# pratyushkumar211/industrial_nnmpc_2021

Hardware: NVIDIA B200
Metric: cdu_closed_loop_sim_steps_per_s (higher is better)
Workload: dtype f64

## Files before the change

industrial_nnmpc_2021_b200/csrc/oz.cu:

```cuda
#include "oz_gemm.cuh"
#include "oz.cuh"
#include "lp.cuh"
#include <cstdlib>
#include <cstring>

namespace nnmpc {

constexpr int OZ_LMAX = 7;
constexpr int OZ_NS = OZ_LMAX + 1;
#ifndef NNMPC_OZ_LMAX_ANCHOR
#define NNMPC_OZ_LMAX_ANCHOR 5
#endif
constexpr int OZ_LMAX_ANCHOR = NNMPC_OZ_LMAX_ANCHOR;

static int oz_variant() {
  static int v = -1;
  if (v < 0) {
    const char* e = getenv("NNMPC_OZ_VARIANT");
    v = e ? atoi(e) : 2;
    if (v < 0 || v > 3) v = 2;
  }
  return v;
}

struct OzEpiStore {
  struct Params {
    double* C;
    long long ldc;
  };
  Params p;
  long long pos;
  __device__ explicit OzEpiStore(const Params& p_) : p(p_), pos(0) {}
  __device__ void begin_row(int pos_, bool) { pos = pos_; }
  __device__ void chunk(int col0, const double (&v)[oz::CH], int N) {
#pragma unroll
    for (int k = 0; k < oz::CH; ++k)
      if (col0 + k < N) p.C[pos * p.ldc + col0 + k] = v[k];
  }
  __device__ void end_row() {}
};

struct OzEpiAnchor {
  struct Params {
    double* X;
    const double* C;
    const int* rows;
    int n;
  };
  Params p;
  long long base;
  __device__ explicit OzEpiAnchor(const Params& p_) : p(p_), base(0) {}
  __device__ void begin_row(int pos, bool ok) { base = ok ? (long long)(p.rows ? p.rows[pos] : pos) * p.n : 0; }
  __device__ void chunk(int col0, const double (&v)[oz::CH], int N) {
    double2 c[oz::CH / 2];
#pragma unroll
    for (int k = 0; k < oz::CH; k += 2) {
      const int col = col0 + k;
      c[k / 2] = make_double2(0.0, 0.0);
      if (col + 1 < N) c[k / 2] = *reinterpret_cast<const double2*>(p.C + base + col);
      else if (col < N) c[k / 2].x = p.C[base + col];
    }
#pragma unroll
    for (int k = 0; k < oz::CH; k += 2) {
      const int col = col0 + k;
      if (col + 1 < N) *reinterpret_cast<double2*>(p.X + base + col) = make_double2(v[k] - c[k / 2].x, v[k + 1] - c[k / 2].y);
      else if (col < N) p.X[base + col] = v[k] - c[k / 2].x;
    }
  }
  __device__ void end_row() {}
};

struct OzEpiVerify {
  struct Params {
    const double* Z;
    const double* Ql;
    const double* lb;
    const double* ub;
    unsigned long long* kres;
    double* G;
    const int* rows;
    int n, nu;
  };
  Params p;
  long long pr;
  bool ok;
  double rmax;
  __device__ explicit OzEpiVerify(const Params& p_) : p(p_), pr(0), ok(false), rmax(0.0) {}
  __device__ void begin_row(int pos, bool ok_) {
    ok = ok_;
    pr = ok ? (long long)(p.rows ? p.rows[pos] : pos) : 0;
    rmax = 0.0;
  }
  __device__ void chunk(int col0, const double (&v)[oz::CH], int N) {
    const long long base = pr * p.n;
    const double* lbr = p.lb + pr * p.nu;
    const double* ubr = p.ub + pr * p.nu;
#pragma unroll
    for (int h = 0; h < oz::CH; h += oz::CH / 2) {
      double z[oz::CH / 2], ql[oz::CH / 2], l[oz::CH / 2], u[oz::CH / 2];
#pragma unroll
      for (int k = 0; k < oz::CH / 2; ++k) {
        const int col = col0 + h + k;
        const bool in = col < N;
        const int s = (in ? col : 0) % p.nu;
        z[k] = in ? p.Z[base + col] : 0.0;
        ql[k] = in ? p.Ql[base + col] : 0.0;
        l[k] = lbr[s];
        u[k] = ubr[s];
      }
#pragma unroll
      for (int k = 0; k < oz::CH / 2; ++k) {
        const int col = col0 + h + k;
        if (col < N) {
          const double g = v[h + k] + ql[k];
          if (p.G) p.G[base + col] = g;
          double r = fabs(z[k] - fmin(fmax(z[k] - g, l[k]), u[k]));
          if (!(r <= 1.7e308)) r = __longlong_as_double(0x7ff0000000000000ll);
          rmax = fmax(rmax, r);
        }
      }
    }
  }
  __device__ void end_row() {
    if (ok) atomicMax(p.kres + pr, (unsigned long long)__double_as_longlong(rmax));
  }
};

int oz_slice_operator(const double* T_dev, int nrows, int ncols, OzOperator* op, cudaStream_t st, long long ld) {
  if (ncols > 32768) return set_error(NNMPC_ERR_BADARG, "oz_slice_operator: contraction length %d above 32768 (int32 accumulators)", ncols);
  op->nrows = nrows; op->ncols = ncols;
  op->ldb = ((long long)ncols + oz::BKB - 1) / oz::BKB * oz::BKB;
  op->rows_pad = ((long long)nrows + 127) / 128 * 128;
  const size_t bytes = (size_t)OZ_NS * op->rows_pad * op->ldb;
  NNMPC_TRY(op->S.ensure(bytes));
  NNMPC_TRY(op->escale.ensure((size_t)op->rows_pad));
  NNMPC_CUDA(cudaMemsetAsync(op->S.p, 0, bytes, st));
  NNMPC_CUDA(cudaMemsetAsync(op->escale.p, 0, (size_t)op->rows_pad * sizeof(double), st));
  oz::k_oz_slice<OZ_NS><<<nrows, 256, 0, st>>>(nullptr, nullptr, T_dev, ld > 0 ? ld : ncols, ncols, op->S.p, op->rows_pad,
                                               op->ldb, op->escale.p, nrows);
  count_launch();
  NNMPC_CUDA(cudaGetLastError());
  if (!oz::make_tmap_u8(&op->tm, op->S.p, OZ_NS * op->rows_pad, op->ldb, op->ldb, oz::BN))
    return set_error(NNMPC_ERR_CUDA, "cuTensorMapEncodeTiled failed for the operator digit planes");
  if (!oz::make_tmap_u8(&op->tm128, op->S.p, OZ_NS * op->rows_pad, op->ldb, op->ldb, 128))
    return set_error(NNMPC_ERR_CUDA, "cuTensorMapEncodeTiled failed for the operator digit planes");
  op->ready = true;
  return 0;
}

int oz_rows_ensure(OzRows* r, long long cap, int ncols, cudaStream_t st, int ns) {
  if (ns <= 0) ns = OZ_NS;
  const long long ldb = ((long long)ncols + oz::BKB - 1) / oz::BKB * oz::BKB;
  const long long cap_pad = (cap + oz::BM - 1) / oz::BM * oz::BM;
  if (cap_pad <= r->cap_pad && ldb == r->ldb && ncols == r->ncols && ns == r->ns) return 0;
  const long long cp = cap_pad > r->cap_pad ? cap_pad : r->cap_pad;
  const size_t bytes = (size_t)ns * cp * ldb;
  NNMPC_TRY(r->S.ensure(bytes));
  NNMPC_TRY(r->fscale.ensure((size_t)cp));
  NNMPC_CUDA(cudaMemsetAsync(r->S.p, 0, bytes, st));
  NNMPC_CUDA(cudaMemsetAsync(r->fscale.p, 0, (size_t)cp * sizeof(double), st));
  if (!oz::make_tmap_u8(&r->tm, r->S.p, ns * cp, ldb, ldb, oz::BM))
    return set_error(NNMPC_ERR_CUDA, "cuTensorMapEncodeTiled failed for the sample digit planes");
  r->cap_pad = cp; r->ldb = ldb; r->ncols = ncols; r->ns = ns;
  return 0;
}

static int oz_slice_rows(OzRows* r, const int* rows, const int* count, int max_rows, const double* src, long long ld_src,
                         cudaStream_t st) {
  if (r->ns == 4 && !rows && !count && r->ncols <= 4096)
    oz::k_oz_slice_warp<4><<<row_grid((max_rows + 7) / 8), 256, 0, st>>>(src, ld_src, r->ncols, r->S.p, r->cap_pad, r->ldb,
                                                                         r->fscale.p, max_rows);
  else if (r->ns == 4)
    oz::k_oz_slice<4><<<row_grid(max_rows), 256, 0, st>>>(rows, count, src, ld_src, r->ncols, r->S.p, r->cap_pad, r->ldb,
                                                          r->fscale.p, max_rows);
  else
    oz::k_oz_slice<OZ_NS><<<row_grid(max_rows), 256, 0, st>>>(rows, count, src, ld_src, r->ncols, r->S.p, r->cap_pad, r->ldb,
                                                              r->fscale.p, max_rows);
  count_launch();
  NNMPC_CUDA(cudaGetLastError());
  return 0;
}

static oz::OzShape oz_shape(const OzOperator* op, const OzRows* r, int max_rows, const int* count) {
  oz::OzShape g{};
  g.M = max_rows; g.N = op->nrows; g.KB = (int)(op->ldb / oz::BKB); g.m_dev = count;
  g.a_rows_pad = r->cap_pad; g.b_rows_pad = op->rows_pad; g.fscale = r->fscale.p; g.escale = op->escale.p;
  g.group_rows = 8;
  return g;
}

template <int LMAX, class Epi>
static int oz_apply(const OzOperator* op, OzRows* r, int max_rows, const int* count, const typename Epi::Params& ep,
                    int device, cudaStream_t st) {
  const int sms = device_sm_count(device);
  const oz::OzShape g = oz_shape(op, r, max_rows, count);
  cudaError_t e;
  const int var = oz_variant();
  if (var == 0) {
    e = oz::launch_oz_gemm<LMAX, Epi>(r->tm, op->tm, g, ep, sms, st);
    count_launch();
  } else if (var == 1) {
    e = oz::launch_oz_gemm2<0, LMAX, 64, Epi>(r->tm, op->tm, oz::OzShape2{g, nullptr, 0, 0}, ep, sms, st);
    count_launch();
  } else {
    NNMPC_TRY(r->partial.ensure((size_t)r->cap_pad * op->nrows));
    e = oz::launch_oz_gemm2<4, LMAX, 128, OzEpiStore>(r->tm, op->tm128, oz::OzShape2{g, nullptr, 0, 1},
                                                      OzEpiStore::Params{r->partial.p, op->nrows}, sms, st);
    if (e == cudaSuccess)
      e = var == 3 ? oz::launch_oz_gemm2<0, 3, 64, Epi>(r->tm, op->tm, oz::OzShape2{g, r->partial.p, op->nrows, 0}, ep, sms, st)
                   : oz::launch_oz_gemm2<0, 3, 128, Epi>(r->tm, op->tm128, oz::OzShape2{g, r->partial.p, op->nrows, 0}, ep, sms, st);
    count_launch(2);
  }
  if (e != cudaSuccess) return set_error(NNMPC_ERR_CUDA, "oz_gemm launch failed: %s", cudaGetErrorString(e));
  return 0;
}

int oz_anchor(const OzOperator* top, OzRows* r, const int* rows, const int* count, int max_rows, const double* W,
              const double* C, double* X, int n, int device, cudaStream_t st) {
  if (max_rows <= 0) return 0;
  if (!top->ready || top->ncols != n || r->ncols != n || max_rows > r->cap_pad)
    return set_error(NNMPC_ERR_BADARG, "oz_anchor: operator / row planes not prepared for n = %d, %d rows", n, max_rows);
  NNMPC_TRY(oz_slice_rows(r, rows, count, max_rows, W, n, st));
  return oz_apply<OZ_LMAX_ANCHOR, OzEpiAnchor>(top, r, max_rows, count, OzEpiAnchor::Params{X, C, rows, n}, device, st);
}

int oz_verify(const OzOperator* P, OzRows* r, const int* rows, const int* count, int max_rows, const double* Z,
              const double* Ql, const double* lb, const double* ub, unsigned long long* kres, double* G, int n, int nu,
              int device, cudaStream_t st) {
  if (max_rows <= 0) return 0;
  if (!P->ready || P->ncols != n || r->ncols != n || max_rows > r->cap_pad)
    return set_error(NNMPC_ERR_BADARG, "oz_verify: operator / row planes not prepared for n = %d, %d rows", n, max_rows);
  NNMPC_TRY(oz_slice_rows(r, rows, count, max_rows, Z, n, st));
  return oz_apply<OZ_LMAX, OzEpiVerify>(P, r, max_rows, count, OzEpiVerify::Params{Z, Ql, lb, ub, kres, G, rows, n, nu},
                                        device, st);
}

struct OzEpiDense {
  struct Params {
    double* out;
    long long ldo;
    const double* bias;
    int relu;
  };
  Params p;
  long long pos;
  __device__ explicit OzEpiDense(const Params& p_) : p(p_), pos(0) {}
  __device__ void begin_row(int pos_, bool) { pos = pos_; }
  __device__ void chunk(int col0, const double (&v)[oz::CH], int N) {
#pragma unroll
    for (int k = 0; k < oz::CH; ++k) {
      const int col = col0 + k;
      if (col < N) {
        double h = v[k] + (p.bias ? __ldg(p.bias + col) : 0.0);
        if (p.relu) h = h > 0.0 ? h : 0.0;
        p.out[pos * p.ldo + col] = h;
      }
    }
  }
  __device__ void end_row() {}
};

int oz_dense_layer(const OzOperator* W, OzRows* r, int M, const double* A, long long lda, const double* bias, int relu,
                   double* out, long long ldo, int device, cudaStream_t st) {
  if (M <= 0) return 0;
  if (!W->ready) return set_error(NNMPC_ERR_BADARG, "oz_dense_layer: weights not sliced");
  NNMPC_TRY(oz_rows_ensure(r, M, W->ncols, st, 4));
  NNMPC_TRY(oz_slice_rows(r, nullptr, nullptr, M, A, lda, st));
  const oz::OzShape g = oz_shape(W, r, M, nullptr);
  cudaError_t e = oz::launch_oz_gemm2<0, 3, 64, OzEpiDense>(r->tm, W->tm, oz::OzShape2{g, nullptr, 0, 0},
                                                            OzEpiDense::Params{out, ldo, bias, relu},
                                                            device_sm_count(device), st);
  count_launch();
  if (e != cudaSuccess) return set_error(NNMPC_ERR_CUDA, "oz_gemm launch failed: %s", cudaGetErrorString(e));
  return 0;
}

struct OzEpiDenseF32 {
  struct Params {
    float* H;
    long long ldh;
    const double* bias;
    float* amax_out;
  };
  Params p;
  long long pos;
  float hmax;
  __device__ explicit OzEpiDenseF32(const Params& p_) : p(p_), pos(0), hmax(0.f) {}
  __device__ void begin_row(int pos_, bool) {
    pos = pos_;
    hmax = 0.f;
  }
  __device__ void chunk(int col0, const double (&v)[oz::CH], int N) {
    __align__(16) float h[oz::CH];
#pragma unroll
    for (int k = 0; k < oz::CH; ++k) {
      double t = 0.0;
      if (col0 + k < N) {
        t = v[k] + __ldg(p.bias + col0 + k);
        t = t > 0.0 ? t : 0.0;
      }
      h[k] = (float)t;
      hmax = fmaxf(hmax, h[k]);
    }
    float4* dst = reinterpret_cast<float4*>(p.H + pos * p.ldh + col0);
#pragma unroll
    for (int q = 0; q < oz::CH / 4; ++q) dst[q] = reinterpret_cast<const float4*>(h)[q];
  }
  __device__ void end_row() {
    atomicMax(reinterpret_cast<unsigned int*>(p.amax_out + pos), __float_as_uint(hmax));
  }
};

__global__ void __launch_bounds__(256)
k_oz_slice_f32(const float* __restrict__ H, long long ldh, int ncols, const float* __restrict__ amax, int8_t* __restrict__ dst,
               long long rows_pad, long long ldb, double* __restrict__ fscale, long long nrows) {
  const int lane = threadIdx.x & 31;
  const long long wpg = (long long)gridDim.x * (blockDim.x >> 5);
  for (long long p = (long long)blockIdx.x * (blockDim.x >> 5) + (threadIdx.x >> 5); p < nrows; p += wpg) {
    const float* a = H + p * ldh;
    const double m = (double)amax[p];
    const bool bad = !(m <= 1.7e308);
    int ex = 0;
    if (!bad && m > 0.0) frexp(m, &ex);
    const double inv = bad ? 0.0 : ldexp(1.0, -(ex + 1));
    for (int k = 4 * lane; k < ncols; k += 128) {
      const float4 f = *reinterpret_cast<const float4*>(a + k);
      double t[4] = {f.x * inv, f.y * inv, f.z * inv, f.w * inv};
#pragma unroll
      for (int s = 0; s < 4; ++s) {
        char4 d;
        int8_t* dd = reinterpret_cast<int8_t*>(&d);
#pragma unroll
        for (int e = 0; e < 4; ++e) {
          t[e] *= 128.0;
          const double r = rint(t[e]);
          t[e] -= r;
          dd[e] = (k + e < ncols) ? (int8_t)(int)r : (int8_t)0;
        }
        *reinterpret_cast<char4*>(dst + ((long long)s * rows_pad + p) * ldb + k) = d;
      }
    }
    if (lane == 0) fscale[p] = bad ? __longlong_as_double(0x7ff8000000000000ll) : ldexp(1.0, ex + 1);
  }
}

int oz_dense_planes(const OzOperator* W, OzRows* rin, int M, const double* bias, OzRows* rout, float* hbuf, long long ldh,
                    float* amax_out, double* out, long long ldo, int device, cudaStream_t st) {
  if (M <= 0) return 0;
  if (!W->ready || rin->ns != 4 || rin->ncols != W->ncols || M > rin->cap_pad)
    return set_error(NNMPC_ERR_BADARG, "oz_dense_planes: operands not prepared");
  const oz::OzShape g = oz_shape(W, rin, M, nullptr);
  cudaError_t e;
  if (out) {
    e = oz::launch_oz_gemm2<0, 3, 64, OzEpiDense>(rin->tm, W->tm, oz::OzShape2{g, nullptr, 0, 0},
                                                  OzEpiDense::Params{out, ldo, bias, 0}, device_sm_count(device), st);
    count_launch();
  } else {
    if (rout->ns != 4 || rout->ncols != W->nrows || M > rout->cap_pad || (ldh & 3) || ldh < ((W->nrows + 63) / 64) * 64)
      return set_error(NNMPC_ERR_BADARG, "oz_dense_planes: output planes / fp32 scratch not prepared");
    e = oz::launch_oz_gemm2<0, 3, 64, OzEpiDenseF32>(rin->tm, W->tm, oz::OzShape2{g, nullptr, 0, 0},
                                                     OzEpiDenseF32::Params{hbuf, ldh, bias, amax_out}, device_sm_count(device), st);
    if (e == cudaSuccess) {
      k_oz_slice_f32<<<row_grid((M + 7) / 8), 256, 0, st>>>(hbuf, ldh, W->nrows, amax_out, rout->S.p, rout->cap_pad, rout->ldb,
                                                            rout->fscale.p, M);
      e = cudaGetLastError();
    }
    count_launch(2);
  }
  if (e != cudaSuccess) return set_error(NNMPC_ERR_CUDA, "oz_gemm launch failed: %s", cudaGetErrorString(e));
  return 0;
}

__global__ void __launch_bounds__(256)
k_oz_pack_network_input(const double* __restrict__ x, const double* __restrict__ uprev, const double* __restrict__ xs,
                        const double* __restrict__ us, const double* __restrict__ xscale, int8_t* __restrict__ dst,
                        long long rows_pad, long long ldb, double* __restrict__ fscale, float* __restrict__ amax, long long B,
                        int nx, int nu, int with_uprev) {
  const int lane = threadIdx.x & 31;
  const long long wpg = (long long)gridDim.x * (blockDim.x >> 5);
  const int o1 = nx, o2 = nx + (with_uprev ? nu : 0), o3 = o2 + nx, o4 = o3 + nu;
  for (long long b = (long long)blockIdx.x * (blockDim.x >> 5) + (threadIdx.x >> 5); b < B; b += wpg) {
    auto value = [&](int c, double& v1, double& v2) {
      if (c < o1) {
        v1 = x[b * nx + c];
        v2 = xs[b * nx + c];
        if (xscale) { v1 /= xscale[c]; v2 /= xscale[c]; }
      } else if (c < o2) {
        v1 = uprev[b * nu + (c - o1)];
        v2 = us[b * nu + (c - o1)];
      } else if (c < o3) {
        v1 = xs[b * nx + (c - o2)];
        if (xscale) v1 /= xscale[c - o2];
        v2 = v1;
      } else {
        v1 = v2 = us[b * nu + (c - o3)];
      }
    };
    double m1 = 0.0, m2 = 0.0;
    for (int c = lane; c < o4; c += 32) {
      double v1, v2;
      value(c, v1, v2);
      const double a1 = fabs(v1), a2 = fabs(v2);
      m1 = (a1 <= m1) ? m1 : a1;
      m2 = (a2 <= m2) ? m2 : a2;
    }
#pragma unroll
    for (int o = 16; o > 0; o >>= 1) {
      const double a1 = __shfl_xor_sync(0xffffffffu, m1, o), a2 = __shfl_xor_sync(0xffffffffu, m2, o);
      m1 = (a1 <= m1) ? m1 : a1;
      m2 = (a2 <= m2) ? m2 : a2;
    }
    double inv[2], fs[2];
    const double mm[2] = {m1, m2};
#pragma unroll
    for (int r = 0; r < 2; ++r) {
      const bool bad = !(mm[r] <= 1.7e308);
      int ex = 0;
      if (!bad && mm[r] > 0.0) frexp(mm[r], &ex);
      inv[r] = bad ? 0.0 : ldexp(1.0, -(ex + 1));
      fs[r] = bad ? __longlong_as_double(0x7ff8000000000000ll) : ldexp(1.0, ex + 1);
    }
    for (int c = lane; c < o4; c += 32) {
      double v1, v2;
      value(c, v1, v2);
      double t1 = v1 * inv[0], t2 = v2 * inv[1];
#pragma unroll
      for (int s = 0; s < 4; ++s) {
        t1 *= 128.0; t2 *= 128.0;
        const double r1 = rint(t1), r2 = rint(t2);
        t1 -= r1; t2 -= r2;
        dst[((long long)s * rows_pad + 2 * b) * ldb + c] = (int8_t)(int)r1;
        dst[((long long)s * rows_pad + 2 * b + 1) * ldb + c] = (int8_t)(int)r2;
      }
    }
    if (lane == 0) {
      fscale[2 * b] = fs[0]; fscale[2 * b + 1] = fs[1];
      amax[2 * b] = (float)m1 * 1.0000002f; amax[2 * b + 1] = (float)m2 * 1.0000002f;
    }
  }
}

int oz_pack_network_input(OzRows* r, long long B, const double* x, const double* uprev, const double* xs, const double* us,
                          const double* xscale, int nx, int nu, int with_uprev, float* amax, cudaStream_t st) {
  if (B <= 0) return 0;
  if (r->ns != 4 || 2 * B > r->cap_pad) return set_error(NNMPC_ERR_BADARG, "oz_pack_network_input: planes not prepared");
  k_oz_pack_network_input<<<row_grid((B + 7) / 8), 256, 0, st>>>(x, uprev, xs, us, xscale, r->S.p, r->cap_pad, r->ldb, r->fscale.p,
                                                                 amax, B, nx, nu, with_uprev);
  count_launch();
  NNMPC_CUDA(cudaGetLastError());
  return 0;
}

}

using namespace nnmpc;

extern "C" {

int nnmpc_oz_gemm_test(int M, int N, int K, const double* A, const double* Bt, double* C, void* stream) {
  if (!A || !Bt || !C || M <= 0 || N <= 0 || K <= 0) return set_error(NNMPC_ERR_BADARG, "nnmpc_oz_gemm_test: bad argument");
  cudaStream_t st = (cudaStream_t)stream;
  int dev = 0;
  NNMPC_CUDA(cudaGetDevice(&dev));
  OzOperator op;
  OzRows rows;
  int rc = oz_slice_operator(Bt, N, K, &op, st);
  if (rc == 0) rc = oz_rows_ensure(&rows, M, K, st);
  if (rc == 0) rc = oz_slice_rows(&rows, nullptr, nullptr, M, A, K, st);
  if (rc == 0) rc = oz_apply<OZ_LMAX, OzEpiStore>(&op, &rows, M, nullptr, OzEpiStore::Params{C, N}, dev, st);
  if (rc == 0 && cudaStreamSynchronize(st) != cudaSuccess)
    rc = set_error(NNMPC_ERR_CUDA, "oz_gemm failed: %s", cudaGetErrorString(cudaGetLastError()));
  cudaStreamSynchronize(st);
  op.release();
  rows.release();
  return rc;
}

int nnmpc_oz_gemm_bench(int M, int N, int K, const double* A, const double* Bt, double* C, int reps, float* ms) {
  if (!A || !Bt || !C || !ms || M <= 0 || N <= 0 || K <= 0 || reps <= 0)
    return set_error(NNMPC_ERR_BADARG, "nnmpc_oz_gemm_bench: bad argument");
  cudaStream_t st = 0;
  int dev = 0;
  NNMPC_CUDA(cudaGetDevice(&dev));
  OzOperator op;
  OzRows rows;
  int rc = oz_slice_operator(Bt, N, K, &op, st);
  if (rc == 0) rc = oz_rows_ensure(&rows, M, K, st);
  cudaEvent_t e0, e1, e2;
  cudaEventCreate(&e0); cudaEventCreate(&e1); cudaEventCreate(&e2);
  for (int w = 0; w < 2 && rc == 0; ++w) {
    rc = oz_slice_rows(&rows, nullptr, nullptr, M, A, K, st);
    if (rc == 0) rc = oz_apply<OZ_LMAX, OzEpiStore>(&op, &rows, M, nullptr, OzEpiStore::Params{C, N}, dev, st);
  }
  if (rc == 0) {
    cudaEventRecord(e0, st);
    for (int i = 0; i < reps && rc == 0; ++i) rc = oz_slice_rows(&rows, nullptr, nullptr, M, A, K, st);
    cudaEventRecord(e1, st);
    for (int i = 0; i < reps && rc == 0; ++i)
      rc = oz_apply<OZ_LMAX, OzEpiStore>(&op, &rows, M, nullptr, OzEpiStore::Params{C, N}, dev, st);
    cudaEventRecord(e2, st);
    if (cudaEventSynchronize(e2) != cudaSuccess) rc = set_error(NNMPC_ERR_CUDA, "oz bench failed: %s", cudaGetErrorString(cudaGetLastError()));
    if (rc == 0) {
      cudaEventElapsedTime(&ms[0], e0, e1);
      cudaEventElapsedTime(&ms[1], e1, e2);
      ms[0] /= reps; ms[1] /= reps;
    }
  }
  cudaEventDestroy(e0); cudaEventDestroy(e1); cudaEventDestroy(e2);
  cudaStreamSynchronize(st);
  op.release();
  rows.release();
  return rc;
}

}
```

industrial_nnmpc_2021_b200/csrc/oz_gemm.cuh:

```cuda
#pragma once
#include "lp_gemm.cuh"

namespace nnmpc {
namespace oz {

constexpr int BM = 128;
constexpr int BN = 64;
constexpr int BKB = 128;
constexpr int UMMA_KB = 32;
constexpr int NS_MAX = 8;
constexpr int A_SLOTS = 4;
constexpr int B_STAGES = 2;
constexpr int A_TILE = BM * BKB;
constexpr int B_TILE = BN * BKB;
constexpr int THREADS = 192;
constexpr int TMEM_COLS = 512;
constexpr int CH = 16;
constexpr int SMEM_BYTES = A_SLOTS * A_TILE + B_STAGES * NS_MAX * B_TILE + 1024 + 256;
static_assert(SMEM_BYTES <= 227 * 1024, "shared memory");

__host__ __device__ constexpr uint32_t make_idesc_i8(int M, int N) {
  return (2u << 4) | (1u << 7) | (1u << 10) | ((uint32_t)(N >> 3) << 17) | ((uint32_t)(M >> 4) << 24);
}
__device__ __forceinline__ void umma_i8(uint32_t tmem_d, uint64_t adesc, uint64_t bdesc, uint32_t idesc, uint32_t accumulate) {
  asm volatile(
      "{\n\t.reg .pred p;\n\t"
      "setp.ne.b32 p, %4, 0;\n\t"
      "tcgen05.mma.cta_group::1.kind::i8 [%0], %1, %2, %3, p;\n\t}"
      ::"r"(tmem_d), "l"(adesc), "l"(bdesc), "r"(idesc), "r"(accumulate)
      : "memory");
}

struct OzShape {
  int M;
  int N;
  int KB;
  const int* m_dev;
  long long a_rows_pad;
  long long b_rows_pad;
  const double* fscale;
  const double* escale;
  int group_rows;
};

__device__ __forceinline__ void oz_tile_coords(int t, int ntm, int ntn, int group_rows, int& bm, int& bn) {
  if (group_rows <= 0 || group_rows >= ntm) {
    bn = t / ntm;
    bm = t - bn * ntm;
    return;
  }
  const int per_group = group_rows * ntn;
  const int gi = t / per_group;
  const int rem = t - gi * per_group;
  const int r0 = gi * group_rows;
  const int gr = (ntm - r0 < group_rows) ? ntm - r0 : group_rows;
  bn = rem / gr;
  bm = r0 + (rem - bn * gr);
}

template <int LMAX, class Epi>
__global__ void __launch_bounds__(THREADS, 1)
oz_gemm_kernel(const __grid_constant__ CUtensorMap tmA, const __grid_constant__ CUtensorMap tmB, OzShape g,
               typename Epi::Params ep) {
  constexpr int NS = LMAX + 1;
  static_assert(NS <= NS_MAX && NS * BN <= TMEM_COLS, "levels");
  extern __shared__ uint8_t smem_raw[];
  uint8_t* base = reinterpret_cast<uint8_t*>((reinterpret_cast<uintptr_t>(smem_raw) + 1023) & ~(uintptr_t)1023);
  uint8_t* a_ring = base;
  uint8_t* b_sets = base + A_SLOTS * A_TILE;
  uint64_t* bars = reinterpret_cast<uint64_t*>(b_sets + B_STAGES * NS_MAX * B_TILE);
  uint64_t* a_full = bars;
  uint64_t* a_empty = a_full + A_SLOTS;
  uint64_t* b_full = a_empty + A_SLOTS;
  uint64_t* b_empty = b_full + B_STAGES;
  uint64_t* acc_full = b_empty + B_STAGES;
  uint64_t* acc_empty = acc_full + 1;
  uint32_t* tmem_slot = reinterpret_cast<uint32_t*>(acc_empty + 1);

  const int warp = threadIdx.x >> 5, lane = threadIdx.x & 31;
  const int M = g.m_dev ? min(*g.m_dev, g.M) : g.M;
  const int ntn = (g.N + BN - 1) / BN;
  const int ntm = (M + BM - 1) / BM;
  const int tiles = ntn * ntm;

  if (warp == 0 && lane == 0) {
    lp::tma_prefetch_desc(&tmA);
    lp::tma_prefetch_desc(&tmB);
    for (int s = 0; s < A_SLOTS; ++s) {
      lp::mbar_init(a_full + s, 1);
      lp::mbar_init(a_empty + s, 1);
    }
    for (int s = 0; s < B_STAGES; ++s) {
      lp::mbar_init(b_full + s, 1);
      lp::mbar_init(b_empty + s, 1);
    }
    lp::mbar_init(acc_full, 1);
    lp::mbar_init(acc_empty, 4);
    lp::fence_barrier_init();
  }
  if (warp == 1) lp::tmem_alloc(tmem_slot, TMEM_COLS);
  lp::tc_fence_before();
  __syncthreads();
  lp::tc_fence_after();
  const uint32_t tmem_base = *tmem_slot;

  if (warp == 0) {
    if (lane == 0) {
      int as = 0, bs = 0;
      uint32_t aph = 0, bph = 0;
      for (int t = blockIdx.x; t < tiles; t += gridDim.x) {
        int bm, bn;
        oz_tile_coords(t, ntm, ntn, g.group_rows, bm, bn);
        for (int kb = 0; kb < g.KB; ++kb) {
          lp::mbar_wait(b_empty + bs, bph ^ 1);
          lp::mbar_expect_tx(b_full + bs, NS * B_TILE);
          for (int j = 0; j < NS; ++j)
            lp::tma_load_2d_hint(b_sets + (bs * NS_MAX + j) * B_TILE, &tmB, b_full + bs, kb * BKB,
                                 (int)(j * g.b_rows_pad) + bn * BN, lp::L2_EVICT_LAST);
          if (++bs == B_STAGES) { bs = 0; bph ^= 1; }
          for (int i = LMAX; i >= 0; --i) {
            lp::mbar_wait(a_empty + as, aph ^ 1);
            lp::mbar_expect_tx(a_full + as, A_TILE);
            lp::tma_load_2d(a_ring + as * A_TILE, &tmA, a_full + as, kb * BKB, (int)(i * g.a_rows_pad) + bm * BM);
            if (++as == A_SLOTS) { as = 0; aph ^= 1; }
          }
        }
      }
    }
  } else if (warp == 1) {
    if (lane == 0) {
      constexpr uint32_t idesc = make_idesc_i8(BM, BN);
      int as = 0, bs = 0;
      uint32_t aph = 0, bph = 0;
      uint32_t tph = 0;
      for (int t = blockIdx.x; t < tiles; t += gridDim.x) {
        lp::mbar_wait(acc_empty, tph ^ 1);
        lp::tc_fence_after();
        for (int kb = 0; kb < g.KB; ++kb) {
          lp::mbar_wait(b_full + bs, bph);
          lp::tc_fence_after();
          const uint32_t sb = lp::smem_u32(b_sets + bs * NS_MAX * B_TILE);
          for (int i = LMAX; i >= 0; --i) {
            lp::mbar_wait(a_full + as, aph);
            lp::tc_fence_after();
            const uint64_t da = lp::make_sw128_kmajor_desc(lp::smem_u32(a_ring + as * A_TILE));
            for (int j = 0; j <= LMAX - i; ++j) {
              const uint64_t db = lp::make_sw128_kmajor_desc(sb + j * B_TILE);
              const uint32_t tacc = tmem_base + (uint32_t)((i + j) * BN);
#pragma unroll
              for (int k = 0; k < BKB / UMMA_KB; ++k)
                umma_i8(tacc, da + 2 * k, db + 2 * k, idesc, (kb | j | k) ? 1u : 0u);
            }
            lp::umma_commit(a_empty + as);
            if (++as == A_SLOTS) { as = 0; aph ^= 1; }
          }
          lp::umma_commit(b_empty + bs);
          if (++bs == B_STAGES) { bs = 0; bph ^= 1; }
        }
        lp::umma_commit(acc_full);
        tph ^= 1;
      }
    }
  } else {
    const int q = warp & 3;
    Epi epi(ep);
    uint32_t tph = 0;
    for (int t = blockIdx.x; t < tiles; t += gridDim.x) {
      int bm, bn;
      oz_tile_coords(t, ntm, ntn, g.group_rows, bm, bn);
      const int pos = bm * BM + q * 32 + lane;
      const bool rok = pos < M;
      const double fs = rok ? g.fscale[pos] : 0.0;
      epi.begin_row(pos, rok);
      lp::mbar_wait(acc_full, tph);
      lp::tc_fence_after();
      const uint32_t trow = tmem_base + ((uint32_t)(q * 32) << 16);
#pragma unroll 1
      for (int c = 0; c < BN / CH; ++c) {
        double v[CH];
#pragma unroll
        for (int k = 0; k < CH; ++k) v[k] = 0.0;
#pragma unroll
        for (int L = LMAX; L >= 0; --L) {
          uint32_t acc[CH];
          lp::tmem_ld_32x16(trow + (uint32_t)(L * BN + c * CH), acc);
          lp::tmem_ld_wait();
#pragma unroll
          for (int k = 0; k < CH; ++k) v[k] = (v[k] + (double)(int)acc[k]) * 0.0078125;
        }
        const int col0 = bn * BN + c * CH;
#pragma unroll
        for (int k = 0; k < CH; ++k) {
          const int col = col0 + k;
          const double es = col < g.N ? g.escale[col] : 0.0;
          v[k] = v[k] * 0.0078125 * fs * es;
        }
        if (rok) epi.chunk(col0, v, g.N);
      }
      epi.end_row();
      lp::tc_fence_before();
      __syncwarp();
      if (lane == 0) lp::mbar_arrive(acc_empty);
      tph ^= 1;
    }
  }

  lp::tc_fence_before();
  __syncthreads();
  if (warp == 1) {
    lp::tc_fence_after();
    lp::tmem_dealloc(tmem_base, TMEM_COLS);
  }
}

constexpr int EPI_WARPS2 = 8;
constexpr int THREADS2 = 64 + 32 * EPI_WARPS2;

template <int BN2_>
struct OzTile2 {
  static constexpr int BN = BN2_;
  static constexpr int B_TILE = BN * BKB;
  static constexpr int A_SLOTS = (BN == 128) ? 5 : 8;
  static constexpr int SMEM_BYTES = A_SLOTS * A_TILE + NS_MAX * B_TILE + 1024 + 512;
  static_assert(SMEM_BYTES <= 227 * 1024, "shared memory");
};

struct OzShape2 {
  OzShape s;
  const double* partial_in;
  long long ldp;
  int raw_out;
};

template <int LLO, int LHI, int BN_, class Epi>
__global__ void __launch_bounds__(THREADS2, 1)
oz_gemm2_kernel(const __grid_constant__ CUtensorMap tmA, const __grid_constant__ CUtensorMap tmB, OzShape2 g2,
                typename Epi::Params ep) {
  using T = OzTile2<BN_>;
  constexpr int BN = T::BN;
  constexpr int NL = LHI - LLO + 1;
  static_assert(LHI < NS_MAX && LLO >= 0 && NL >= 1 && NL * BN <= TMEM_COLS, "level window");
  constexpr int NSB = LHI + 1;
  constexpr bool DB = 2 * NSB <= NS_MAX;
  constexpr int ACC = (2 * NL * BN <= TMEM_COLS) ? 2 : 1;
  auto b_slot = [](int j, uint32_t kbc) -> int { return DB ? (int)(kbc & 1u) * NSB + j : j; };
  auto b_par = [](uint32_t kbc) -> uint32_t { return DB ? (kbc >> 1) & 1u : kbc & 1u; };
  const OzShape& g = g2.s;
  extern __shared__ uint8_t smem_raw[];
  uint8_t* base = reinterpret_cast<uint8_t*>((reinterpret_cast<uintptr_t>(smem_raw) + 1023) & ~(uintptr_t)1023);
  uint8_t* a_ring = base;
  uint8_t* b_slots = base + T::A_SLOTS * A_TILE;
  uint64_t* bars = reinterpret_cast<uint64_t*>(b_slots + NS_MAX * T::B_TILE);
  uint64_t* a_full = bars;
  uint64_t* a_empty = a_full + T::A_SLOTS;
  uint64_t* b_full = a_empty + T::A_SLOTS;
  uint64_t* b_empty = b_full + NS_MAX;
  uint64_t* acc_full = b_empty + NS_MAX;
  uint64_t* acc_empty = acc_full + 2;
  uint32_t* tmem_slot = reinterpret_cast<uint32_t*>(acc_empty + 2);

  const int warp = threadIdx.x >> 5, lane = threadIdx.x & 31;
  const int M = g.m_dev ? min(*g.m_dev, g.M) : g.M;
  const int ntn = (g.N + BN - 1) / BN;
  const int ntm = (M + BM - 1) / BM;
  const int tiles = ntn * ntm;

  if (warp == 0 && lane == 0) {
    lp::tma_prefetch_desc(&tmA);
    lp::tma_prefetch_desc(&tmB);
    for (int s = 0; s < T::A_SLOTS; ++s) {
      lp::mbar_init(a_full + s, 1);
      lp::mbar_init(a_empty + s, 1);
    }
    for (int s = 0; s < NS_MAX; ++s) {
      lp::mbar_init(b_full + s, 1);
      lp::mbar_init(b_empty + s, 1);
    }
    for (int s = 0; s < ACC; ++s) {
      lp::mbar_init(acc_full + s, 1);
      lp::mbar_init(acc_empty + s, EPI_WARPS2);
    }
    lp::fence_barrier_init();
  }
  if (warp == 1) lp::tmem_alloc(tmem_slot, TMEM_COLS);
  lp::tc_fence_before();
  __syncthreads();
  lp::tc_fence_after();
  const uint32_t tmem_base = *tmem_slot;

  if (warp == 0) {
    if (lane == 0) {
      int as = 0;
      uint32_t aph = 0, kbc = 0;
      for (int t = blockIdx.x; t < tiles; t += gridDim.x) {
        int bm, bn;
        oz_tile_coords(t, ntm, ntn, g.group_rows, bm, bn);
        for (int kb = 0; kb < g.KB; ++kb, ++kbc) {
          const uint32_t bph = b_par(kbc);
          for (int i = 0; i <= LHI; ++i) {
            lp::mbar_wait(a_empty + as, aph ^ 1);
            lp::mbar_expect_tx(a_full + as, A_TILE);
            lp::tma_load_2d(a_ring + as * A_TILE, &tmA, a_full + as, kb * BKB, (int)(i * g.a_rows_pad) + bm * BM);
            if (++as == T::A_SLOTS) { as = 0; aph ^= 1; }
            const int jhi = (i == 0) ? LHI : LLO - i;
            const int jlo = (i == 0) ? LLO : LLO - i;
            for (int j = jhi; j >= jlo && j >= 0; --j) {
              const int sl = b_slot(j, kbc);
              lp::mbar_wait(b_empty + sl, bph ^ 1);
              lp::mbar_expect_tx(b_full + sl, T::B_TILE);
              lp::tma_load_2d_hint(b_slots + sl * T::B_TILE, &tmB, b_full + sl, kb * BKB, (int)(j * g.b_rows_pad) + bn * BN,
                                   lp::L2_EVICT_LAST);
            }
          }
        }
      }
    }
  } else if (warp == 1) {
    constexpr uint32_t idesc = make_idesc_i8(BM, BN);
    const bool issue = lane == 0;
    int as = 0;
    uint32_t aph = 0, kbc = 0, ti = 0;
    const uint64_t da_base = lp::make_sw128_kmajor_desc(lp::smem_u32(a_ring));
    const uint64_t db_base = lp::make_sw128_kmajor_desc(lp::smem_u32(b_slots));
    for (int t = blockIdx.x; t < tiles; t += gridDim.x, ++ti) {
      const uint32_t acs = ACC == 2 ? (ti & 1u) : 0u;
      const uint32_t tph = ACC == 2 ? (ti >> 1) & 1u : ti & 1u;
      lp::mbar_wait(acc_empty + acs, tph ^ 1);
      lp::tc_fence_after();
      for (int kb = 0; kb < g.KB; ++kb, ++kbc) {
        const uint32_t first = kb ? 1u : 0u;
        const uint32_t bph = b_par(kbc);
        const int sbase = DB ? (int)(kbc & 1u) * NSB : 0;
#pragma unroll
        for (int i = 0; i <= LHI; ++i) {
          lp::mbar_wait(a_full + as, aph);
          lp::tc_fence_after();
          const uint64_t da = da_base + (uint64_t)(as * (A_TILE >> 4));
#pragma unroll
          for (int j = LHI - i; j >= (LLO - i > 0 ? LLO - i : 0); --j) {
            if (i == (LLO - j > 0 ? LLO - j : 0)) {
              lp::mbar_wait(b_full + sbase + j, bph);
              lp::tc_fence_after();
            }
            const uint64_t db = db_base + (uint64_t)((sbase + j) * (T::B_TILE >> 4));
            const uint32_t tacc = tmem_base + (uint32_t)((acs * NL + (i + j - LLO)) * BN);
            if (issue) {
              umma_i8(tacc, da, db, idesc, i == 0 ? first : 1u);
              umma_i8(tacc, da + 2, db + 2, idesc, 1u);
              umma_i8(tacc, da + 4, db + 4, idesc, 1u);
              umma_i8(tacc, da + 6, db + 6, idesc, 1u);
            }
          }
          if (issue) {
            lp::umma_commit(a_empty + as);
            lp::umma_commit(b_empty + sbase + (LHI - i));
          }
          __syncwarp();
          if (++as == T::A_SLOTS) { as = 0; aph ^= 1; }
        }
      }
      if (issue) lp::umma_commit(acc_full + acs);
      __syncwarp();
    }
  } else {
    const int q = warp & 3;
    const int hsel = (warp - 2) >> 2;
    constexpr int CHUNKS = BN / CH / 2;
    Epi epi(ep);
    uint32_t ti = 0;
    const double lev0 = __longlong_as_double((long long)(1023 - 7 * (LLO + 1)) << 52);
    for (int t = blockIdx.x; t < tiles; t += gridDim.x, ++ti) {
      const uint32_t acs = ACC == 2 ? (ti & 1u) : 0u;
      const uint32_t tph = ACC == 2 ? (ti >> 1) & 1u : ti & 1u;
      int bm, bn;
      oz_tile_coords(t, ntm, ntn, g.group_rows, bm, bn);
      const int pos = bm * BM + q * 32 + lane;
      const bool rok = pos < M;
      const double fs = rok ? g.fscale[pos] : 0.0;
      epi.begin_row(pos, rok);
      lp::mbar_wait(acc_full + acs, tph);
      lp::tc_fence_after();
      const uint32_t trow = tmem_base + ((uint32_t)(q * 32) << 16) + (uint32_t)(acs * NL * BN);
#pragma unroll 1
      for (int c = hsel * CHUNKS; c < (hsel + 1) * CHUNKS; ++c) {
        double v[CH];
        const int colc = bn * BN + c * CH;
        double pin[CH], es[CH];
        {
          const bool vec_ok = colc + CH <= g.N && (!g2.partial_in || (g2.ldp & 1) == 0);
          const bool has_p = g2.partial_in && rok;
          const double* pp = g2.partial_in + (has_p ? (long long)pos * g2.ldp + colc : 0);
#pragma unroll
          for (int k = 0; k < CH; k += 2) {
            double2 t = make_double2(0.0, 0.0), e2 = make_double2(0.0, 0.0);
            if (vec_ok) {
              if (has_p) t = *reinterpret_cast<const double2*>(pp + k);
              if (!g2.raw_out) e2 = *reinterpret_cast<const double2*>(g.escale + colc + k);
            } else {
              if (has_p && colc + k < g.N) t.x = pp[k];
              if (has_p && colc + k + 1 < g.N) t.y = pp[k + 1];
              if (!g2.raw_out && colc + k < g.N) e2.x = g.escale[colc + k];
              if (!g2.raw_out && colc + k + 1 < g.N) e2.y = g.escale[colc + k + 1];
            }
            pin[k] = t.x; pin[k + 1] = t.y;
            es[k] = e2.x; es[k + 1] = e2.y;
          }
        }
        if constexpr (NL <= 4) {
          long long sacc[CH];
#pragma unroll
          for (int k = 0; k < CH; ++k) sacc[k] = 0;
#pragma unroll
          for (int L = 0; L < NL; ++L) {
            uint32_t acc[CH];
            lp::tmem_ld_32x16(trow + (uint32_t)(L * BN + c * CH), acc);
            lp::tmem_ld_wait();
#pragma unroll
            for (int k = 0; k < CH; ++k) sacc[k] = sacc[k] * 128 + (long long)(int)acc[k];
          }
          const double wnl = __longlong_as_double((long long)(1023 - 7 * (NL + LLO + 1)) << 52);
#pragma unroll
          for (int k = 0; k < CH; ++k) v[k] = (double)sacc[k] * wnl;
        } else {
#pragma unroll
          for (int k = 0; k < CH; ++k) v[k] = 0.0;
#pragma unroll
          for (int L = NL - 1; L >= 0; --L) {
            uint32_t acc[CH];
            lp::tmem_ld_32x16(trow + (uint32_t)(L * BN + c * CH), acc);
            lp::tmem_ld_wait();
#pragma unroll
            for (int k = 0; k < CH; ++k) v[k] = (v[k] + (double)(int)acc[k]) * 0.0078125;
          }
#pragma unroll
          for (int k = 0; k < CH; ++k) v[k] *= lev0;
        }
        const int col0 = colc;
#pragma unroll
        for (int k = 0; k < CH; ++k) {
          v[k] += pin[k];
          if (!g2.raw_out) v[k] *= fs * es[k];
        }
        if (rok) epi.chunk(col0, v, g.N);
      }
      epi.end_row();
      lp::tc_fence_before();
      __syncwarp();
      if (lane == 0) lp::mbar_arrive(acc_empty + acs);
    }
  }

  lp::tc_fence_before();
  __syncthreads();
  if (warp == 1) {
    lp::tc_fence_after();
    lp::tmem_dealloc(tmem_base, TMEM_COLS);
  }
}

template <int LLO, int LHI, int BN_, class Epi>
inline cudaError_t launch_oz_gemm2(const CUtensorMap& tmA, const CUtensorMap& tmB, const OzShape2& g,
                                   const typename Epi::Params& ep, int num_sms, cudaStream_t st) {
  using T = OzTile2<BN_>;
  static bool configured[64] = {};
  int dev = 0;
  cudaGetDevice(&dev);
  if (!configured[dev & 63]) {
    cudaError_t e = cudaFuncSetAttribute(oz_gemm2_kernel<LLO, LHI, BN_, Epi>, cudaFuncAttributeMaxDynamicSharedMemorySize,
                                         T::SMEM_BYTES);
    if (e != cudaSuccess) return e;
    configured[dev & 63] = true;
  }
  if (g.s.M <= 0 || g.s.N <= 0 || g.s.KB <= 0) return cudaSuccess;
  const long long tiles = (long long)((g.s.N + T::BN - 1) / T::BN) * ((g.s.M + BM - 1) / BM);
  const unsigned grid = (unsigned)(tiles < num_sms ? tiles : num_sms);
  oz_gemm2_kernel<LLO, LHI, BN_, Epi><<<grid, THREADS2, T::SMEM_BYTES, st>>>(tmA, tmB, g, ep);
  return cudaGetLastError();
}

template <int NS>
__global__ void __launch_bounds__(256)
k_oz_slice(const int* __restrict__ rows, const int* __restrict__ count, const double* __restrict__ src, long long ld_src,
           int ncols, int8_t* __restrict__ dst, long long rows_pad, long long ldb, double* __restrict__ scale_out,
           int max_rows) {
  const long long total = count ? (*count < max_rows ? *count : max_rows) : (long long)max_rows;
  __shared__ double red[8];
  for (long long p = blockIdx.x; p < total; p += gridDim.x) {
    const long long r = rows ? rows[p] : p;
    const double* a = src + r * ld_src;
    double m = 0.0;
    for (int k = threadIdx.x; k < ncols; k += blockDim.x) {
      const double b = fabs(a[k]);
      m = (b <= m) ? m : b;
    }
#pragma unroll
    for (int o = 16; o > 0; o >>= 1) {
      const double b = __shfl_xor_sync(0xffffffffu, m, o);
      m = (b <= m) ? m : b;
    }
    if ((threadIdx.x & 31) == 0) red[threadIdx.x >> 5] = m;
    __syncthreads();
    m = red[0];
    for (int w = 1; w < 8; ++w) m = (red[w] <= m) ? m : red[w];
    __syncthreads();
    const bool bad = !(m <= 1.7e308);
    int ex = 0;
    if (!bad && m > 0.0) frexp(m, &ex);
    const double inv = bad ? 0.0 : ldexp(1.0, -(ex + 1));
    for (int k = threadIdx.x; k < ncols; k += blockDim.x) {
      double t = bad ? 0.0 : a[k] * inv;
#pragma unroll
      for (int s = 0; s < NS; ++s) {
        t *= 128.0;
        const double d = rint(t);
        t -= d;
        dst[((long long)s * rows_pad + p) * ldb + k] = (int8_t)(int)d;
      }
    }
    if (threadIdx.x == 0)
      scale_out[p] = bad ? __longlong_as_double(0x7ff8000000000000ll) : ldexp(1.0, ex + 1);
  }
}

template <int NS>
__global__ void __launch_bounds__(256)
k_oz_slice_warp(const double* __restrict__ src, long long ld_src, int ncols, int8_t* __restrict__ dst, long long rows_pad,
                long long ldb, double* __restrict__ scale_out, long long nrows) {
  const int lane = threadIdx.x & 31;
  const long long wpg = (long long)gridDim.x * (blockDim.x >> 5);
  for (long long p = (long long)blockIdx.x * (blockDim.x >> 5) + (threadIdx.x >> 5); p < nrows; p += wpg) {
    const double* a = src + p * ld_src;
    double m = 0.0;
    for (int k = lane; k < ncols; k += 32) {
      const double b = fabs(a[k]);
      m = (b <= m) ? m : b;
    }
#pragma unroll
    for (int o = 16; o > 0; o >>= 1) {
      const double b = __shfl_xor_sync(0xffffffffu, m, o);
      m = (b <= m) ? m : b;
    }
    const bool bad = !(m <= 1.7e308);
    int ex = 0;
    if (!bad && m > 0.0) frexp(m, &ex);
    const double inv = bad ? 0.0 : ldexp(1.0, -(ex + 1));
    const int n4 = ncols & ~3;
    for (int k = 4 * lane; k < n4; k += 128) {
      double t[4];
#pragma unroll
      for (int e = 0; e < 4; ++e) t[e] = bad ? 0.0 : a[k + e] * inv;
#pragma unroll
      for (int s = 0; s < NS; ++s) {
        char4 d;
        int8_t* dd = reinterpret_cast<int8_t*>(&d);
#pragma unroll
        for (int e = 0; e < 4; ++e) {
          t[e] *= 128.0;
          const double r = rint(t[e]);
          t[e] -= r;
          dd[e] = (int8_t)(int)r;
        }
        *reinterpret_cast<char4*>(dst + ((long long)s * rows_pad + p) * ldb + k) = d;
      }
    }
    for (int k = n4 + lane; k < ncols; k += 32) {
      double t = bad ? 0.0 : a[k] * inv;
#pragma unroll
      for (int s = 0; s < NS; ++s) {
        t *= 128.0;
        const double r = rint(t);
        t -= r;
        dst[((long long)s * rows_pad + p) * ldb + k] = (int8_t)(int)r;
      }
    }
    if (lane == 0) scale_out[p] = bad ? __longlong_as_double(0x7ff8000000000000ll) : ldexp(1.0, ex + 1);
  }
}

inline bool make_tmap_u8(CUtensorMap* tm, const void* base, long long rows, long long cols, long long ld, int box_rows) {
  lp::EncodeTiledFn fn = lp::encode_tiled_fn();
  if (!fn) return false;
  cuuint64_t dims[2] = {(cuuint64_t)cols, (cuuint64_t)rows};
  cuuint64_t strides[1] = {(cuuint64_t)ld};
  cuuint32_t box[2] = {(cuuint32_t)BKB, (cuuint32_t)box_rows};
  cuuint32_t estr[2] = {1, 1};
  CUresult r = fn(tm, CU_TENSOR_MAP_DATA_TYPE_UINT8, 2, const_cast<void*>(base), dims, strides, box, estr,
                  CU_TENSOR_MAP_INTERLEAVE_NONE, CU_TENSOR_MAP_SWIZZLE_128B, CU_TENSOR_MAP_L2_PROMOTION_L2_256B,
                  CU_TENSOR_MAP_FLOAT_OOB_FILL_NONE);
  return r == CUDA_SUCCESS;
}

template <int LMAX, class Epi>
inline cudaError_t launch_oz_gemm(const CUtensorMap& tmA, const CUtensorMap& tmB, const OzShape& g,
                                  const typename Epi::Params& ep, int num_sms, cudaStream_t st) {
  static bool configured[64] = {};
  int dev = 0;
  cudaGetDevice(&dev);
  if (!configured[dev & 63]) {
    cudaError_t e = cudaFuncSetAttribute(oz_gemm_kernel<LMAX, Epi>, cudaFuncAttributeMaxDynamicSharedMemorySize, SMEM_BYTES);
    if (e != cudaSuccess) return e;
    configured[dev & 63] = true;
  }
  if (g.M <= 0 || g.N <= 0 || g.KB <= 0) return cudaSuccess;
  const long long tiles = (long long)((g.N + BN - 1) / BN) * ((g.M + BM - 1) / BM);
  const unsigned grid = (unsigned)(tiles < num_sms ? tiles : num_sms);
  oz_gemm_kernel<LMAX, Epi><<<grid, THREADS, SMEM_BYTES, st>>>(tmA, tmB, g, ep);
  return cudaGetLastError();
}

}
}
```

Baseline: 232,500.

## Fuse high- and low-level Ozaki int8 GEMM passes into one persistent kernel

Adds a fused Ozaki-scheme kernel that computes the high-level slice products and then the low-level slice products for each tile within one warp-specialized persistent kernel. Partial sums stay in registers between the two phases instead of being written to a global partial buffer and read back by a second launch. It uses 384 threads with setmaxnreg register rebalancing and makes this the default variant. This removes one kernel launch and a global round trip per GEMM, at the cost of a longer and more complex pipeline per tile and higher register pressure in the epilogue warps.

```diff
diff --git a/industrial_nnmpc_2021_b200/csrc/oz.cu b/industrial_nnmpc_2021_b200/csrc/oz.cu
--- a/industrial_nnmpc_2021_b200/csrc/oz.cu
+++ b/industrial_nnmpc_2021_b200/csrc/oz.cu
@@ -17,8 +17,8 @@
   static int v = -1;
   if (v < 0) {
     const char* e = getenv("NNMPC_OZ_VARIANT");
-    v = e ? atoi(e) : 2;
-    if (v < 0 || v > 3) v = 2;
+    v = e ? atoi(e) : 4;
+    if (v < 0 || v > 4) v = 4;
   }
   return v;
 }
@@ -201,6 +201,9 @@
     count_launch();
   } else if (var == 1) {
     e = oz::launch_oz_gemm2<0, LMAX, 64, Epi>(r->tm, op->tm, oz::OzShape2{g, nullptr, 0, 0}, ep, sms, st);
+    count_launch();
+  } else if (var == 4) {
+    e = oz::launch_oz_fused<LMAX, Epi>(r->tm, op->tm128, g, ep, sms, st);
     count_launch();
   } else {
     NNMPC_TRY(r->partial.ensure((size_t)r->cap_pad * op->nrows));
diff --git a/industrial_nnmpc_2021_b200/csrc/oz_gemm.cuh b/industrial_nnmpc_2021_b200/csrc/oz_gemm.cuh
--- a/industrial_nnmpc_2021_b200/csrc/oz_gemm.cuh
+++ b/industrial_nnmpc_2021_b200/csrc/oz_gemm.cuh
@@ -478,6 +478,299 @@
   return cudaGetLastError();
 }
 
+constexpr int THREADS_F = 384;
+constexpr int FUSED_REGS_LAUNCH = (65536 / THREADS_F) & ~7;
+constexpr int FUSED_REGS_LO = 48;
+constexpr int FUSED_REGS_HI = 224;
+static_assert(128 * FUSED_REGS_LO + 256 * FUSED_REGS_HI <= THREADS_F * FUSED_REGS_LAUNCH, "register pool of the block");
+
+template <int LMAX, class Epi>
+__global__ void __launch_bounds__(THREADS_F, 1)
+oz_fused_kernel(const __grid_constant__ CUtensorMap tmA, const __grid_constant__ CUtensorMap tmB, OzShape g,
+                typename Epi::Params ep) {
+  using T = OzTile2<128>;
+  constexpr int BN = T::BN;
+  constexpr int LLO = 4;
+  constexpr int NLH = LMAX - LLO + 1;
+  static_assert(LMAX < NS_MAX && NLH >= 1 && NLH <= LLO && LLO * BN <= TMEM_COLS, "level windows");
+  constexpr int HALF = BN / 2;
+  constexpr int NCH = HALF / CH;
+  auto lo_base = [](int kb) -> int { return (kb & 1) ? 0 : LLO; };
+  extern __shared__ uint8_t smem_raw[];
+  uint8_t* base = reinterpret_cast<uint8_t*>((reinterpret_cast<uintptr_t>(smem_raw) + 1023) & ~(uintptr_t)1023);
+  uint8_t* a_ring = base;
+  uint8_t* b_slots = base + T::A_SLOTS * A_TILE;
+  uint64_t* bars = reinterpret_cast<uint64_t*>(b_slots + NS_MAX * T::B_TILE);
+  uint64_t* a_full = bars;
+  uint64_t* a_empty = a_full + T::A_SLOTS;
+  uint64_t* b_full = a_empty + T::A_SLOTS;
+  uint64_t* b_empty = b_full + NS_MAX;
+  uint64_t* acc_full = b_empty + NS_MAX;
+  uint64_t* acc_empty = acc_full + 1;
+  uint32_t* tmem_slot = reinterpret_cast<uint32_t*>(acc_empty + 1);
+
+  const int warp = threadIdx.x >> 5, lane = threadIdx.x & 31;
+  const int M = g.m_dev ? min(*g.m_dev, g.M) : g.M;
+  const int ntn = (g.N + BN - 1) / BN;
+  const int ntm = (M + BM - 1) / BM;
+  const int tiles = ntn * ntm;
+
+  if (warp == 0 && lane == 0) {
+    lp::tma_prefetch_desc(&tmA);
+    lp::tma_prefetch_desc(&tmB);
+    for (int s = 0; s < T::A_SLOTS; ++s) {
+      lp::mbar_init(a_full + s, 1);
+      lp::mbar_init(a_empty + s, 1);
+    }
+    for (int s = 0; s < NS_MAX; ++s) {
+      lp::mbar_init(b_full + s, 1);
+      lp::mbar_init(b_empty + s, 1);
+    }
+    lp::mbar_init(acc_full, 1);
+    lp::mbar_init(acc_empty, EPI_WARPS2);
+    lp::fence_barrier_init();
+  }
+  if (warp == 1) lp::tmem_alloc(tmem_slot, TMEM_COLS);
+  lp::tc_fence_before();
+  __syncthreads();
+  lp::tc_fence_after();
+  const uint32_t tmem_base = *tmem_slot;
+
+  if (warp < 4) {
+    asm volatile("setmaxnreg.dec.sync.aligned.u32 %0;" ::"n"(FUSED_REGS_LO));
+  }
+  if (warp == 0) {
+    if (lane == 0) {
+      int as = 0;
+      uint32_t aph = 0, bpar = 0;
+      auto load_a = [&](int kb, int i, int bm) {
+        lp::mbar_wait(a_empty + as, aph ^ 1);
+        lp::mbar_expect_tx(a_full + as, A_TILE);
+        lp::tma_load_2d(a_ring + as * A_TILE, &tmA, a_full + as, kb * BKB, (int)(i * g.a_rows_pad) + bm * BM);
+        if (++as == T::A_SLOTS) { as = 0; aph ^= 1; }
+      };
+      auto load_b = [&](int kb, int j, int sl, int bn) {
+        lp::mbar_wait(b_empty + sl, ((bpar >> sl) & 1u) ^ 1u);
+        lp::mbar_expect_tx(b_full + sl, T::B_TILE);
+        lp::tma_load_2d_hint(b_slots + sl * T::B_TILE, &tmB, b_full + sl, kb * BKB, (int)(j * g.b_rows_pad) + bn * BN,
+                             lp::L2_EVICT_LAST);
+        bpar ^= 1u << sl;
+      };
+      for (int t = blockIdx.x; t < tiles; t += gridDim.x) {
+        int bm, bn;
+        oz_tile_coords(t, ntm, ntn, g.group_rows, bm, bn);
+        for (int kb = 0; kb < g.KB; ++kb) {
+          for (int i = 0; i <= LMAX; ++i) {
+            load_a(kb, i, bm);
+            if (i == 0)
+              for (int j = LMAX; j >= LLO; --j) load_b(kb, j, j, bn);
+            else if (i <= LLO)
+              load_b(kb, LLO - i, LLO - i, bn);
+          }
+        }
+        for (int kb = 0; kb < g.KB; ++kb) {
+          load_a(kb, 0, bm);
+          for (int j = LLO - 1; j >= 0; --j) load_b(kb, j, lo_base(kb) + j, bn);
+          for (int i = 1; i < LLO; ++i) load_a(kb, i, bm);
+        }
+      }
+    }
+  } else if (warp == 1) {
+    constexpr uint32_t idesc = make_idesc_i8(BM, BN);
+    const bool issue = lane == 0;
+    int as = 0;
+    uint32_t aph = 0, bpar = 0, aph_acc = 0;
+    const uint64_t da_base = lp::make_sw128_kmajor_desc(lp::smem_u32(a_ring));
+    const uint64_t db_base = lp::make_sw128_kmajor_desc(lp::smem_u32(b_slots));
+    auto wait_a = [&]() -> uint32_t {
+      lp::mbar_wait(a_full + as, aph);
+      lp::tc_fence_after();
+      return (uint32_t)da_base + (uint32_t)(as * (A_TILE >> 4));
+    };
+    auto release_a = [&]() {
+      if (issue) lp::umma_commit(a_empty + as);
+      if (++as == T::A_SLOTS) { as = 0; aph ^= 1; }
+    };
+    auto wait_b = [&](int sl) {
+      lp::mbar_wait(b_full + sl, (bpar >> sl) & 1u);
+      lp::tc_fence_after();
+      bpar ^= 1u << sl;
+    };
+    auto mma4 = [&](int level, uint32_t da_lo, int sl, uint32_t acc0) {
+      uint32_t db_lo = (uint32_t)db_base + (uint32_t)(sl * (T::B_TILE >> 4));
+      asm volatile("" : "+r"(da_lo), "+r"(db_lo));
+      const uint64_t da = (da_base & 0xffffffff00000000ull) | da_lo;
+      const uint64_t db = (db_base & 0xffffffff00000000ull) | db_lo;
+      const uint32_t tacc = tmem_base + (uint32_t)(level * BN);
+      if (issue) {
+        umma_i8(tacc, da, db, idesc, acc0);
+        umma_i8(tacc, da + 2, db + 2, idesc, 1u);
+        umma_i8(tacc, da + 4, db + 4, idesc, 1u);
+        umma_i8(tacc, da + 6, db + 6, idesc, 1u);
+      }
+    };
+    for (int t = blockIdx.x; t < tiles; t += gridDim.x) {
+      lp::mbar_wait(acc_empty, aph_acc ^ 1);
+      lp::tc_fence_after();
+      aph_acc ^= 1;
+      for (int kb = 0; kb < g.KB; ++kb) {
+        const uint32_t first = kb ? 1u : 0u;
+#pragma unroll
+        for (int i = 0; i <= LMAX; ++i) {
+          const uint32_t da = wait_a();
+#pragma unroll
+          for (int j = LMAX - i; j >= (LLO - i > 0 ? LLO - i : 0); --j) {
+            if (i == (LLO - j > 0 ? LLO - j : 0)) wait_b(j);
+            mma4(i + j - LLO, da, j, i == 0 ? first : 1u);
+          }
+          if (issue) lp::umma_commit(b_empty + (LMAX - i));
+          release_a();
+          __syncwarp();
+        }
+      }
+      if (issue) lp::umma_commit(acc_full);
+      __syncwarp();
+      lp::mbar_wait(acc_empty, aph_acc ^ 1);
+      lp::tc_fence_after();
+      aph_acc ^= 1;
+      for (int kb = 0; kb < g.KB; ++kb) {
+        const uint32_t first = kb ? 1u : 0u;
+        const int sb = lo_base(kb);
+#pragma unroll
+        for (int i = 0; i < LLO; ++i) {
+          const uint32_t da = wait_a();
+#pragma unroll
+          for (int j = LLO - 1 - i; j >= 0; --j) {
+            if (i == 0) wait_b(sb + j);
+            mma4(i + j, da, sb + j, i == 0 ? first : 1u);
+          }
+          if (issue) lp::umma_commit(b_empty + sb + (LLO - 1 - i));
+          release_a();
+          __syncwarp();
+        }
+      }
+      if (issue) lp::umma_commit(acc_full);
+      __syncwarp();
+    }
+  } else if (warp >= 4) {
+    asm volatile("setmaxnreg.inc.sync.aligned.u32 %0;" ::"n"(FUSED_REGS_HI));
+    const int q = warp & 3;
+    const int hsel = (warp - 4) >> 2;
+    Epi epi(ep);
+    uint32_t aph_acc = 0;
+    const double w_hi = __longlong_as_double((long long)(1023 - 7 * (NLH + LLO + 1)) << 52);
+    const double w_lo = __longlong_as_double((long long)(1023 - 7 * (LLO + 1)) << 52);
+    for (int t = blockIdx.x; t < tiles; t += gridDim.x) {
+      int bm, bn;
+      oz_tile_coords(t, ntm, ntn, g.group_rows, bm, bn);
+      const int pos = bm * BM + q * 32 + lane;
+      const bool rok = pos < M;
+      const uint32_t trow = tmem_base + ((uint32_t)(q * 32) << 16) + (uint32_t)(hsel * HALF);
+      double v[NCH][CH];
+      lp::mbar_wait(acc_full, aph_acc);
+      lp::tc_fence_after();
+      aph_acc ^= 1;
+#pragma unroll
+      for (int c = 0; c < NCH; ++c) {
+        long long sacc[CH];
+#pragma unroll
+        for (int k = 0; k < CH; ++k) sacc[k] = 0;
+#pragma unroll
+        for (int L = 0; L < NLH; ++L) {
+          uint32_t acc[CH];
+          lp::tmem_ld_32x16(trow + (uint32_t)(L * BN + c * CH), acc);
+          lp::tmem_ld_wait();
+#pragma unroll
+          for (int k = 0; k < CH; ++k) sacc[k] = sacc[k] * 128 + (long long)(int)acc[k];
+        }
+#pragma unroll
+        for (int k = 0; k < CH; ++k) v[c][k] = (double)sacc[k] * w_hi;
+      }
+      lp::tc_fence_before();
+      __syncwarp();
+      if (lane == 0) lp::mbar_arrive(acc_empty);
+      const double fs = rok ? g.fscale[pos] : 0.0;
+      epi.begin_row(pos, rok);
+      lp::mbar_wait(acc_full, aph_acc);
+      lp::tc_fence_after();
+      aph_acc ^= 1;
+#pragma unroll
+      for (int c = 0; c < NCH; ++c) {
+#pragma unroll
+        for (int h = 0; h < CH; h += CH / 2) {
+          long long sacc[CH / 2];
+#pragma unroll
+          for (int k = 0; k < CH / 2; ++k) sacc[k] = 0;
+#pragma unroll
+          for (int L = 0; L < LLO; ++L) {
+            uint32_t acc[CH / 2];
+            lp::tmem_ld_32x8(trow + (uint32_t)(L * BN + c * CH + h), acc);
+            lp::tmem_ld_wait();
+#pragma unroll
+            for (int k = 0; k < CH / 2; ++k) sacc[k] = sacc[k] * 128 + (long long)(int)acc[k];
+          }
+          const int colc = bn * BN + hsel * HALF + c * CH + h;
+          double es[CH / 2];
+          const bool vec_ok = colc + CH / 2 <= g.N;
+#pragma unroll
+          for (int k = 0; k < CH / 2; k += 2) {
+            double2 e2 = make_double2(0.0, 0.0);
+            if (vec_ok) {
+              e2 = *reinterpret_cast<const double2*>(g.escale + colc + k);
+            } else {
+              if (colc + k < g.N) e2.x = g.escale[colc + k];
+              if (colc + k + 1 < g.N) e2.y = g.escale[colc + k + 1];
+            }
+            es[k] = e2.x; es[k + 1] = e2.y;
+          }
+#pragma unroll
+          for (int k = 0; k < CH / 2; ++k) {
+            double x = (double)sacc[k] * w_lo;
+            x += v[c][h + k];
+            x *= fs * es[k];
+            v[c][h + k] = x;
+          }
+        }
+      }
+      lp::tc_fence_before();
+      __syncwarp();
+      if (lane == 0) lp::mbar_arrive(acc_empty);
+      if (rok) {
+#pragma unroll
+        for (int c = 0; c < NCH; ++c) epi.chunk(bn * BN + hsel * HALF + c * CH, v[c], g.N);
+      }
+      epi.end_row();
+    }
+  }
+
+  lp::tc_fence_before();
+  __syncthreads();
+  if (warp == 1) {
+    lp::tc_fence_after();
+    lp::tmem_dealloc(tmem_base, TMEM_COLS);
+  }
+}
+
+template <int LMAX, class Epi>
+inline cudaError_t launch_oz_fused(const CUtensorMap& tmA, const CUtensorMap& tmB, const OzShape& g,
+                                   const typename Epi::Params& ep, int num_sms, cudaStream_t st) {
+  using T = OzTile2<128>;
+  static bool configured[64] = {};
+  int dev = 0;
+  cudaGetDevice(&dev);
+  if (!configured[dev & 63]) {
+    cudaError_t e = cudaFuncSetAttribute(oz_fused_kernel<LMAX, Epi>, cudaFuncAttributeMaxDynamicSharedMemorySize,
+                                         T::SMEM_BYTES);
+    if (e != cudaSuccess) return e;
+    configured[dev & 63] = true;
+  }
+  if (g.M <= 0 || g.N <= 0 || g.KB <= 0) return cudaSuccess;
+  const long long tiles = (long long)((g.N + T::BN - 1) / T::BN) * ((g.M + BM - 1) / BM);
+  const unsigned grid = (unsigned)(tiles < num_sms ? tiles : num_sms);
+  oz_fused_kernel<LMAX, Epi><<<grid, THREADS_F, T::SMEM_BYTES, st>>>(tmA, tmB, g, ep);
+  return cudaGetLastError();
+}
+
 template <int NS>
 __global__ void __launch_bounds__(256)
 k_oz_slice(const int* __restrict__ rows, const int* __restrict__ count, const double* __restrict__ src, long long ld_src,
```

Result: faster. 236,300 (median of 6 runs) (+1.6%).
